# linghaosong/Sextans

Measured on AMD Instinct MI355X. Metric: SpMM GFLOP/s + achieved HBM GB/s (fp32, N=16) at 1/2/4/8 MI355X, higher is better.
Workload: dtype f32; 1 GPU; config4: synthetic CSR 4000000x4000000, Poisson(40) nnz/row, U(-1,1) fp32, N=16, alpha=0.85, beta=-2.06, column-major B/C, seed 4; M=4000000, K=4000000, N=16, nnz=159999547, parallelism=1 GPU

## Files before the change

sextans_amd/csrc/engine.hip:

```cpp
#include <algorithm>
#include <cstdlib>
#include <cstring>

#include "engine_launch.h"
#include "window_plan.h"

namespace sxe {
thread_local std::string g_last_error;
}
using namespace sxe;

namespace sxe {

int check_device(int device) {
    int n = 0;
    if (hipGetDeviceCount(&n) != hipSuccess || n <= 0) {
        g_last_error = "hipGetDeviceCount: no HIP device";
        return SEXTANS_ERR_NO_DEVICE;
    }
    if (device < 0 || device >= n) return SEXTANS_ERR_INVALID;
    hipDeviceProp_t p;
    if (hipGetDeviceProperties(&p, device) != hipSuccess) return SEXTANS_ERR_NO_DEVICE;
    if (strncmp(p.gcnArchName, "gfx950", 6) != 0) {
        g_last_error = std::string("device is ") + p.gcnArchName + ", engine is built for gfx950 only";
        return SEXTANS_ERR_NO_DEVICE;
    }
    return SEXTANS_OK;
}

enum Drops { kNothing, kWindowStream, kClusterPlan, kPackedPlans, kColwiseVerdict };
constexpr int64_t kMin = INT64_MIN, kMax = INT64_MAX;
using E = sextans_engine;
static const struct Option {
    const char *key; int64_t E::*slot; Drops drops = kNothing; bool measurement = false; int64_t lo = kMin, hi = kMax; uint64_t only = 0;
} kOptions[] = {
    {"kernel", &E::opt_kernel}, {"stage_a", &E::opt_stage}, {"xcd_remap", &E::opt_xcd}, {"exact", &E::opt_exact}, {"profile", &E::opt_profile},
    {"split_rows", &E::opt_split_rows}, {"bucket_rows", &E::opt_bucket_rows}, {"global_nnz", &E::opt_global_nnz}, {"exact_chain", &E::opt_exact_chain},
    {"fuse_b", &E::opt_fuse_b}, {"small_v2", &E::opt_small_v2}, {"colwise_tiles_adjacent", &E::opt_colwise_tiles_adjacent}, {"window_auto", &E::opt_win_auto},
    {"bell_wide", &E::opt_bell_wide}, {"bell_generation", &E::opt_bell_gen}, {"bell_shared", &E::opt_bell_shared}, {"mfma_dense_tiles", &E::opt_mfma_dense},
    {"dense_tile_fill_x100", &E::opt_dense_fill_x100},
    {"lanes_per_row", &E::opt_lpr, kNothing, false, kMin, kMax, 1 | 1 << 2 | 1 << 4 | 1 << 8},
    {"cols_per_lane", &E::opt_cols_per_lane, kNothing, false, kMin, kMax, 1 | 1 << 4 | 1 << 8},
    {"window_unroll", &E::opt_win_unroll, kNothing, false, kMin, kMax, 1 << 4 | 1 << 8},
    {"tiles_per_wg", &E::opt_tiles_per_wg, kNothing, false, 0, 1024}, {"panel_v2", &E::opt_panel_v2, kNothing, false, -1, 1},
    {"phase_timing", &E::opt_phase_timing, kNothing, true}, {"reordered_xcd", &E::opt_reordered_xcd, kNothing, true}, {"bell_debug", &E::opt_bell_debug, kNothing, true},
    {"dist_broadcast_runs", &E::opt_dist_broadcast_runs, kNothing, true}, {"rowblock_tiles", &E::opt_rb_tiles, kNothing, true},
    {"cluster_shape", &E::opt_cluster_shape, kClusterPlan, true},
    {"cluster_group", &E::opt_cluster_group, kClusterPlan, true, 1, 64},
    {"panel_min_reuse_x100", &E::opt_min_reuse_x100, kClusterPlan}, {"panel_min_reuse_wide_x100", &E::opt_min_reuse_wide_x100, kClusterPlan},
    {"row_cluster", &E::opt_row_cluster, kClusterPlan, false, -1, 2}, {"row_similarity", &E::opt_row_similarity, kClusterPlan, false, -1, 1},
    {"cluster_top", &E::opt_cluster_top, kClusterPlan}, {"small_panel", &E::opt_small_panel, kClusterPlan}, {"row_sets", &E::opt_row_sets, kClusterPlan},
    {"row_offset", &E::opt_row_offset, kClusterPlan}, {"relabel_columns", &E::opt_relabel_columns, kClusterPlan}, {"run_cluster", &E::opt_run_cluster, kClusterPlan},
    {"refine_sweeps", &E::opt_refine_sweeps, kClusterPlan}, {"refine_rows", &E::opt_refine_rows, kClusterPlan},
    {"window_rows", &E::opt_win_rows, kWindowStream, false, 1, sx::kWinMaxRowsPerWave}, {"window_cols", &E::opt_win_cols, kWindowStream, false, 1, 0x7fffffff},
    {"share_index", &E::opt_share_index, kPackedPlans}, {"split_mixed", &E::opt_split_mixed, kPackedPlans},
    {"colwise_max_len", &E::opt_colwise_max_len, kColwiseVerdict},
};

static const Option *find_option(const char *key) {
    for (const Option &o : kOptions)
        if (!strcmp(key, o.key)) return &o;
    return nullptr;
}

int transposed_options(sextans_engine *h, const char *key, int64_t value) {
    auto skip = [](const char *k) { return !strcmp(k, "row_offset") || !strcmp(k, "global_nnz"); };
    if (key) return skip(key) ? SEXTANS_OK : sextans_set_option(h->tr, key, value);
    for (const auto &o : kOptions)
        if (!skip(o.key) && h->tr->*o.slot != h->*o.slot)
            if (int rc = sextans_set_option(h->tr, o.key, h->*o.slot)) return rc;
    h->tr->opt_mode = h->opt_mode;
    return SEXTANS_OK;
}

}

extern "C" {

const char *sextans_last_error(void) { return g_last_error.c_str(); }

int sextans_device_count(int *count) {
    if (!count) return SEXTANS_ERR_INVALID;
    *count = 0;
    int n = 0;
    if (hipGetDeviceCount(&n) != hipSuccess || n <= 0) return SEXTANS_ERR_NO_DEVICE;
    int ok = 0;
    for (int d = 0; d < n; ++d)
        if (check_device(d) == SEXTANS_OK) ++ok;
    *count = ok;
    return ok > 0 ? SEXTANS_OK : SEXTANS_ERR_NO_DEVICE;
}

int sextans_create(sextans_handle_t *out, int device) {
    if (!out) return SEXTANS_ERR_INVALID;
    *out = nullptr;
    if (int rc = check_device(device)) return rc;
    SX_HIP(hipSetDevice(device));
    auto *h = new sextans_engine();
    h->device = device;
    {
        hipDeviceProp_t p;
        if (hipGetDeviceProperties(&p, device) == hipSuccess && p.multiProcessorCount > 0)
            h->num_cus = p.multiProcessorCount;
    }
    preload_device_code();
    *out = h;
    return SEXTANS_OK;
}

int sextans_destroy(sextans_handle_t h) {
    if (!h) return SEXTANS_ERR_INVALID;
    (void)hipSetDevice(h->device);
    free_matrix(h);
    free_bell(h);
    (void)hipFree(h->d_bell_Bf);
    (void)hipFree(h->d_Bp); (void)hipFree(h->d_B); (void)hipFree(h->d_Cin); (void)hipFree(h->d_Cout); (void)hipFree(h->d_Cs);
    sextans_profile_reset(h);
    (void)hipFree(h->d_P);
    if (h->ev_fork) (void)hipEventDestroy(h->ev_fork);
    if (h->ev_join) (void)hipEventDestroy(h->ev_join);
    if (h->aux_stream) (void)hipStreamDestroy(h->aux_stream);
    (void)hipFree(h->d_dbg);
    (void)hipFree(h->d_chB); (void)hipFree(h->d_chC);
    (void)hipFree(h->d_stage);
    (void)hipFree(h->d_Cfull); (void)hipFree(h->d_dist_rows); (void)hipFree(h->d_rmB); (void)hipFree(h->d_rmC);
    for (hipEvent_t e : h->dist_events) (void)hipEventDestroy(e);
    if (h->comm_stream) (void)hipStreamDestroy(h->comm_stream);
// ... 129 lines not shown
    for (int i = threadIdx.x; i < np; i += 64) {
        const int c = dict[(int64_t)(b - 1) * stride + i];
        unsigned s = ((unsigned)c * 2654435761u) >> 22;
        while (atomicCAS(&tab[s], -1, c) != -1 && tab[s] != c) s = (s + 1) & 1023u;
    }
    __syncthreads();
    unsigned found = 0;
    for (int i = threadIdx.x; i < nc; i += 64) {
        const int c = dict[(int64_t)b * stride + i];
        unsigned s = ((unsigned)c * 2654435761u) >> 22;
        while (tab[s] != -1 && tab[s] != c) s = (s + 1) & 1023u;
        found += tab[s] == c;
    }
    for (int o = 32; o > 0; o >>= 1) found += __shfl_down(found, o);
    if (threadIdx.x == 0) { atomicAdd(&out[0], (unsigned long long)found); atomicAdd(&out[1], (unsigned long long)nc); }
}
int run16_stat(sextans_engine *h, double *value) {
    *value = 0.0;
    if (h->cluster_state <= 0 || !h->d_slot_row || h->psc.plan_nblk <= 0) return SEXTANS_OK;
    const int RB = kBlock / 4 * std::max(1, h->psc.plan_sets);
    std::vector<int> sr((size_t)h->psc.plan_nblk * RB);
    SX_HIP(hipMemcpy(sr.data(), h->d_slot_row, sizeof(int) * sr.size(), hipMemcpyDeviceToHost));
    const std::vector<int> &br = h->psc.h_blk_row;
    if ((int)br.size() != h->psc.plan_nblk + 1) return SEXTANS_OK;
    int64_t in_runs = 0, slots = 0;
    for (int b = 0; b < h->psc.plan_nblk; ++b) {
        const int n = br[(size_t)b + 1] - br[(size_t)b];
        const int *r = sr.data() + (size_t)b * RB;
        slots += n;
        for (int i = 0; i < n;) {
            int j = i + 1;
            while (j < n && r[j] == r[j - 1] + 1) ++j;
            if (j - i >= 16) in_runs += j - i;
            i = j;
        }
    }
    *value = slots ? (double)in_runs / (double)slots : 0.0;
    return SEXTANS_OK;
}
int dict_overlap_stat(sextans_engine *h, double *value) {
    const sextans_engine::PanelState &P = h->cluster_state > 0 ? h->psc : h->ps;
    *value = 0.0;
    if (!P.plan_built || P.plan_nblk < 2 || !P.d_dict || !P.d_dict_ptr) return SEXTANS_OK;
    unsigned long long *d = nullptr, hv[2] = {0, 0};
    SX_HIP(hipMalloc((void **)&d, sizeof hv));
    SX_HIP(hipMemset(d, 0, sizeof hv));
    hipLaunchKernelGGL(dict_overlap, dim3((unsigned)P.plan_nblk - 1), dim3(64), 0, hipStreamPerThread, P.d_dict_ptr, P.d_dict, P.plan_dict_stride, P.plan_nblk, d);
    const hipError_t e = hipMemcpy(hv, d, sizeof hv, hipMemcpyDeviceToHost);
    (void)hipFree(d);
    SX_HIP(e);
    *value = hv[1] ? (double)hv[0] / (double)hv[1] : 0.0;
    return SEXTANS_OK;
}
}
extern "C" {

int sextans_get_stat(sextans_handle_t h, const char *key, double *value) {
    if (!h || !key || !value) return SEXTANS_ERR_INVALID;
    if (h->d_rp) {
        SX_HIP(hipSetDevice(h->device));
        if (int rc = ensure_dense(h)) return rc;
        if (int rc = ensure_split(h)) return rc;
    }
    if (!strcmp(key, "plan_build_s")) *value = h->plan_build_s;
    else if (!strcmp(key, "window_padded_entries")) *value = (double)h->win_padded;
    else if (!strcmp(key, "window_state")) *value = (double)h->win_state;
    else if (!strcmp(key, "reassociated_rows")) *value = (double)h->h_split_rows.size();
    else if (!strcmp(key, "piece_path_rows")) *value = (double)(h->nhub + h->nchain);
    else if (!strcmp(key, "exact_chain_rows")) *value = (double)h->nchain;
    else if (!strcmp(key, "chain_threshold")) *value = (double)h->chain_T;
    else if (!strcmp(key, "split_threshold")) *value = (double)h->split_T;
    else if (!strcmp(key, "bucket_threshold")) *value = (double)h->bucket_L0;
    else if (!strcmp(key, "dense_tiles")) *value = (double)h->dense_tiles;
    else if (!strcmp(key, "dense_tile_fraction")) *value = h->nnz > 0 ? (double)h->dense_nnz / (double)h->nnz : 0.0;
    else if (!strcmp(key, "dense_tiles_on_mfma")) *value = h->dense_W > 0 ? 1.0 : 0.0;
    else if (!strcmp(key, "bell_share")) *value = h->bell_share;
    else if (!strcmp(key, "row_cluster")) *value = (double)h->cluster_state;
    else if (!strcmp(key, "cluster_shared_fraction")) *value = h->cluster_shared;
    else if (!strcmp(key, "cluster_decline")) *value = (double)h->cluster_decline;
    else if (!strcmp(key, "graph_fallbacks")) *value = (double)h->graph_fallbacks;
    else if (!strcmp(key, "cluster_run16_fraction")) return run16_stat(h, value);
    else if (!strcmp(key, "dict_overlap_consecutive")) return dict_overlap_stat(h, value);
    else if (!strcmp(key, "dist_setup_exchanges")) *value = (double)h->dist_exchanges;
    else if (!strcmp(key, "cluster_graph_kind")) *value = (double)h->cluster_graph_kind;
    else if (!strcmp(key, "cluster_runs")) *value = h->cluster_runs ? 1.0 : 0.0;
    else if (!strcmp(key, "pattern_symmetry")) *value = h->pattern_symmetry;
    else if (!strcmp(key, "col_range_lo")) *value = (double)h->col_lo;
    else if (!strcmp(key, "col_range_hi")) *value = (double)h->col_hi;
    else if (!strcmp(key, "b_rows_repacked")) *value = h->d_touched ? (double)h->touched_segments * 64.0 : (double)(h->col_hi - h->col_lo);
    else if (!strcmp(key, "colwise")) *value = (double)h->colwise_state;
    else if (!strcmp(key, "mixed_plan")) *value = h->ps.plan_built && h->ps.plan_mixed ? (h->ps.d_rg_skip && h->opt_split_mixed != 0 ? 2.0 : 1.0) : 0.0;
    else if (!strcmp(key, "row_sets")) *value = (double)(h->cluster_state > 0 ? h->psc.plan_sets : h->ps.plan_sets);
    else if (!strcmp(key, "row_coherence")) *value = h->row_coherence;
    else if (!strcmp(key, "panel_blocks_clustered")) *value = (double)h->psc.plan_nblk;
    else if (!strcmp(key, "device_bytes")) *value = (double)device_bytes(h);
    else if (!strcmp(key, "softmax_long_rows")) *value = (double)h->sm_long_rows;
    else if (!strcmp(key, "value_refreshes")) *value = (double)h->value_refreshes;
    else if (!strcmp(key, "value_refresh_rebuilt")) *value = (double)h->value_refresh_rebuilt;
    else if (!strcmp(key, "bf16_native_calls")) *value = (double)(h->bf16_native_calls + (h->tr ? h->tr->bf16_native_calls : 0));
    else if (!strcmp(key, "bf16_converted_calls")) *value = (double)(h->bf16_converted_calls + (h->tr ? h->tr->bf16_converted_calls : 0));
    else if (!strcmp(key, "transpose_build_s")) *value = h->transpose_build_s + (h->tr ? h->tr->plan_build_s : 0.0);
    else if (!strcmp(key, "grid_stride_line")) *value = (double)h->cluster_s2;
    else if (!strcmp(key, "grid_stride_plane")) *value = (double)h->cluster_s3;
    else if (!strcmp(key, "panel_rows_natural")) *value = (double)h->plan_total_dict;
    else if (!strcmp(key, "panel_rows_clustered")) *value = (double)h->cluster_total_dict;
    else if (!strcmp(key, "panel_fraction")) *value = h->ps.plan_panel_frac;
    else if (!strcmp(key, "panel_blocks")) *value = (double)h->ps.plan_nblk;
    else if (!strcmp(key, "index_stream_entries")) *value = (double)(h->cluster_state > 0 ? h->psc.plan_idx_len : h->ps.plan_idx_len);
    else if (!strcmp(key, "value_stream_entries")) *value = (double)(h->cluster_state > 0 ? h->psc.plan_stream_len : h->ps.plan_stream_len);
    else return SEXTANS_ERR_INVALID;
    return SEXTANS_OK;
}

int sextans_export_plan(sextans_handle_t h, int lanes_per_row, sextans_packed *out) {
    if (!h || !out || (lanes_per_row != 2 && lanes_per_row != 4 && lanes_per_row != 8)) return SEXTANS_ERR_INVALID;
    if (!h->d_rp) return SEXTANS_ERR_STATE;
    SX_HIP(hipSetDevice(h->device));
    if (int rc = ensure_dense(h)) return rc;
    if (int rc = ensure_split(h)) return rc;
    if (int rc = ensure_plan(h, lanes_per_row, true)) return rc;
    if (!h->ps.plan_built) return SEXTANS_ERR_STATE;
    if (int rc = restore_plan_streams(h)) return rc;
    const auto &ps = h->ps;
    const int M = h->M, nblk = ps.plan_nblk, RB = kBlock / lanes_per_row;
    const size_t L = (size_t)ps.plan_stream_len;
    memset(out, 0, sizeof *out);
    out->M = M; out->K = h->K; out->nnz = h->m_nnz; out->lanes_per_row = lanes_per_row; out->nblk = nblk;
    out->stream_len = (int64_t)L; out->max_dict = ps.plan_max_dict; out->nnz_in_panel_blocks = ps.plan_nnz_panel;
    std::vector<int> rp((size_t)M + 1), cnt((size_t)nblk), bd((size_t)nblk * ps.plan_dict_stride);
    SX_HIP(hipMemcpy(rp.data(), h->m_rp, sizeof(int) * rp.size(), hipMemcpyDeviceToHost));
    if (nblk) {
        SX_HIP(hipMemcpy(cnt.data(), ps.d_dict_ptr, sizeof(int) * cnt.size(), hipMemcpyDeviceToHost));
        SX_HIP(hipMemcpy(bd.data(), ps.d_dict, sizeof(int) * bd.size(), hipMemcpyDeviceToHost));
    }
#define SX_HIP_OUT(call) do { if ((call) != hipSuccess) { g_last_error = #call; (void)hipGetLastError(); sextans_packed_free(out); return SEXTANS_ERR_HIP; } } while (0)
    auto alloc = [](size_t bytes) { return calloc(bytes ? bytes : 1, 1); };
    out->blk_row = (int *)alloc(sizeof(int) * ((size_t)nblk + 1));
    out->dict_ptr = (int *)alloc(sizeof(int) * ((size_t)nblk + 1));
    out->row_off = (int *)alloc(sizeof(int) * ((size_t)M + 1));
    out->idx16 = (uint16_t *)alloc(sizeof(uint16_t) * L);
    out->col32 = (int *)alloc(sizeof(int) * L);
    out->val = (float *)alloc(sizeof(float) * L);
    size_t ndict = 0;
    for (int b = 0; b < nblk; ++b) ndict += (size_t)cnt[(size_t)b];
    out->dict = (int *)alloc(sizeof(int) * ndict);
    if (!out->blk_row || !out->dict_ptr || !out->row_off || !out->idx16 || !out->col32 || !out->val || !out->dict) {
        sextans_packed_free(out);
        return SEXTANS_ERR_ALLOC;
    }
    memcpy(out->blk_row, ps.h_blk_row.data(), sizeof(int) * ((size_t)nblk + 1));
    size_t w = 0;
    for (int b = 0; b < nblk; ++b) {
        out->dict_ptr[b] = (int)w;
        for (int i = 0; i < cnt[(size_t)b]; ++i) out->dict[w++] = bd[(size_t)b * ps.plan_dict_stride + (size_t)i];
    }
    out->dict_ptr[nblk] = (int)w;
    for (int r = 0; r < M; ++r) out->row_off[r + 1] = out->row_off[r] + ((rp[(size_t)r + 1] - rp[(size_t)r] + 3) & ~3);
    if (!ps.d_ioff) {
        SX_HIP_OUT(hipMemcpy(out->idx16, ps.d_lidx, sizeof(uint16_t) * L, hipMemcpyDeviceToHost));
    } else {
        std::vector<uint16_t> comp((size_t)ps.plan_idx_len);
        std::vector<int> ioff((size_t)nblk * RB * 2), sinfo((size_t)nblk * RB * 2);
        SX_HIP_OUT(hipMemcpy(comp.data(), ps.d_lidx, sizeof(uint16_t) * comp.size(), hipMemcpyDeviceToHost));
        SX_HIP_OUT(hipMemcpy(ioff.data(), ps.d_ioff, sizeof(int) * ioff.size(), hipMemcpyDeviceToHost));
        SX_HIP_OUT(hipMemcpy(sinfo.data(), ps.d_row_off, sizeof(int) * sinfo.size(), hipMemcpyDeviceToHost));
        const unsigned pad = (unsigned)ps.plan_pad_row * 16u * (unsigned)lanes_per_row;
// ... 113 lines not shown
```

sextans_amd/csrc/engine_dist.hip:

```cpp
#include <dlfcn.h>

#include <algorithm>
#include <cstring>
#include <mutex>

#include "engine_launch.h"

using namespace sxe;

namespace sxe {
namespace {
__global__ __launch_bounds__(256) void position_rows(int nblk, int RB, const int *__restrict__ blk_row, const int *__restrict__ slot_row, int row0, int *__restrict__ out) {
    const int b = blockIdx.x, s = threadIdx.x;
    if (b >= nblk || s >= RB) return;
    const int p0 = blk_row[b], n = blk_row[b + 1] - p0;
    if (s < n) out[p0 + s] = slot_row[(int64_t)b * RB + s] + row0;
}
}

static bool cc_usable(sextans_engine *h, int N, const Tiling &t) {
    return h->cluster_state == 2 && h->cluster_cm_pays && t.W == 16 && N % 16 == 0 && t.segs.size() == 1 && t.segs[0].width == 16 && h->nhub == 0 &&
           h->nchain == 0 && csr_only(h) && (h->opt_kernel == 0 || h->opt_kernel == 2) && h->d_Cs && h->d_slot_row &&
           h->Cs_cap >= (size_t)(N / 16) * (size_t)h->M * 16 && h->Bp_cap >= (size_t)h->K * (size_t)N && h->psc.plan_sets == 1 &&
           (h->M >= 65536 || h->m_nnz * (int64_t)N >= ((int64_t)24 << 20)) && (int)h->psc.h_blk_row.size() == h->psc.plan_nblk + 1;
// ... 98 lines not shown
    if (i < m.y) C[(int64_t)m.x + i + (int64_t)n * ldc] = S[((int64_t)g * N + n) * lmax + i];
}

int exchange(sextans_engine *h, Rccl *r, void *comm, int world, int rank, const int *mine, int n, std::vector<int> &all, int status, hipStream_t s,
             const char *what) {
    ++h->dist_exchanges;
    const size_t per = (size_t)n + 1;
    std::vector<int> me(per, 0), buf(per * (size_t)world, 0);
    for (int i = 0; i < n; ++i) me[(size_t)i] = status ? 0 : mine[i];
    me[(size_t)n] = status;
    int *d = nullptr;
    SX_HIP(hipMalloc((void **)&d, sizeof(int) * buf.size()));
    hipError_t e0 = hipMemcpyAsync(d + per * (size_t)rank, me.data(), sizeof(int) * per, hipMemcpyHostToDevice, s);
    const int rc = e0 != hipSuccess ? SEXTANS_OK : rccl_check(r->AllGather(d + per * (size_t)rank, d, per, 2 , comm, s), what);
    hipError_t e1 = (rc || e0 != hipSuccess) ? hipSuccess : hipMemcpyAsync(buf.data(), d, sizeof(int) * buf.size(), hipMemcpyDeviceToHost, s);
    hipError_t e2 = hipStreamSynchronize(s);
    (void)hipFree(d);
    if (rc) return rc;
    SX_HIP(e0);
    SX_HIP(e1);
    SX_HIP(e2);
    bool peer_failed = false;
    all.assign((size_t)n * (size_t)world, 0);
    for (int g = 0; g < world; ++g) {
        peer_failed = peer_failed || buf[per * (size_t)g + (size_t)n] != 0;
        for (int i = 0; i < n; ++i) all[(size_t)g * n + (size_t)i] = buf[per * (size_t)g + (size_t)i];
    }
    if (status) return status;
    if (peer_failed) {
        g_last_error = std::string(what) + ": another rank reported a failure";
        return SEXTANS_ERR_PEER;
    }
    return SEXTANS_OK;
}

struct Partition {
    int64_t M_total = 0;
    int row0 = 0, m_loc = 0, m_max = 0;
    bool equal = true;
};
int read_partition(int world, int rank, const int *row_ranges, int multiple_of, Partition &p) {
    p = Partition();
    for (int g = 0; g < world; ++g) {
        if (row_ranges[2 * g] != (int)p.M_total || row_ranges[2 * g + 1] < row_ranges[2 * g] || (row_ranges[2 * g + 1] % multiple_of)) return SEXTANS_ERR_INVALID;
        p.M_total = row_ranges[2 * g + 1];
        p.m_max = std::max(p.m_max, row_ranges[2 * g + 1] - row_ranges[2 * g]);
        p.equal = p.equal && row_ranges[2 * g + 1] - row_ranges[2 * g] == row_ranges[1] - row_ranges[0];
    }
    p.row0 = row_ranges[2 * rank];
    p.m_loc = row_ranges[2 * rank + 1] - p.row0;
    return SEXTANS_OK;
}

int exchange_nnz(sextans_engine *h, Rccl *r, void *comm, int world, int rank, const int *row_ranges, bool force, int status, hipStream_t s, bool *exchanged) {
    if (!comm) return status;
    std::vector<int> nnz_key(row_ranges, row_ranges + 2 * world);
    nnz_key.push_back(rank);
    if (!force && h->dist_nnz_key == nnz_key) return status;
    const int mine_nz[2] = {(int)(h->nnz & 0x7fffffff), (int)(h->nnz >> 31)};
    std::vector<int> all_nz;
    *exchanged = true;
    if (int rc = exchange(h, r, comm, world, rank, mine_nz, 2, all_nz, status, s, "ncclAllGather(nnz)")) return rc;
    int64_t total = 0;
    for (int g = 0; g < world; ++g) total += (int64_t)all_nz[2 * (size_t)g] + ((int64_t)all_nz[2 * (size_t)g + 1] << 31);
    if (total != h->opt_global_nnz)
        if (int rc = sextans_set_option(h, "global_nnz", total)) return rc;
    h->dist_nnz_key = nnz_key;
    return SEXTANS_OK;
}

int settle(sextans_engine *h, Rccl *r, void *comm, int world, int rank, int status, bool exchanged, hipStream_t s) {
    if (!comm || !exchanged) return status;
    std::vector<int> none;
    const int rc = exchange(h, r, comm, world, rank, nullptr, 0, none, status, s, "ncclAllGather(status)");
    if (rc) { h->dist_cut_key.clear(); h->dist_nnz_key.clear(); }
    return rc;
}

struct CmSetup {
    Partition p;
    std::vector<int64_t> lmax, off;
    int *d_meta = nullptr;
    bool cc = false;
};
int setup_cm(sextans_engine *h, Rccl *r, void *comm, int world, int rank, const int *row_ranges, int N, int &nchunks, hipStream_t s, bool force, CmSetup &out) {
    bool exchanged = false;
    int st = read_partition(world, rank, row_ranges, 1, out.p);
    const Partition &p = out.p;
    if (!st && p.m_loc != h->M) st = SEXTANS_ERR_INVALID;
    if (!st && !h->d_rp) st = SEXTANS_ERR_STATE;
    if (st && !(force && comm)) return st;
    if (!st && world > 1 && h->opt_row_offset != p.row0) st = sextans_set_option(h, "row_offset", p.row0);
    if (nchunks < 1) nchunks = 1;
    if (nchunks > 16) nchunks = 16;
    if (int rc = exchange_nnz(h, r, comm, world, rank, row_ranges, force, st, s, &exchanged)) return rc;
    bool want_cc = false;
    if (nchunks > 1) {
        st = cc_prepare(h, N, &want_cc);
    } else if (h->M > 0) {
        st = prepare(h, N);
    }
    if (want_cc && h->psc.plan_nblk < nchunks) want_cc = false;
    std::vector<int> key(row_ranges, row_ranges + 2 * world);
    key.push_back(N); key.push_back(nchunks); key.push_back(rank); key.push_back(want_cc ? 1 : 0);
    if (force || h->dist_cut_key != key || st) {
        h->dist_cut_key.clear();
        const size_t need = (size_t)world * (size_t)p.m_max;
        if (!st && want_cc && h->dist_rows_cap < need) {
            (void)hipFree(h->d_dist_rows);
            h->d_dist_rows = nullptr; h->dist_rows_cap = 0;
            if (hipMalloc((void **)&h->d_dist_rows, sizeof(int) * std::max<size_t>(need, 1)) != hipSuccess) { (void)hipGetLastError(); st = SEXTANS_ERR_HIP; g_last_error = "hipMalloc(row tables) failed"; }
            else h->dist_rows_cap = need;
        }
        bool all_cc = want_cc && !st;
        if (comm) {
            const int mine_f = want_cc ? 1 : 0;
            std::vector<int> f;
            exchanged = true;
            if (int rc = exchange(h, r, comm, world, rank, &mine_f, 1, f, st, s, "ncclAllGather(mode)")) return rc;
            for (int g = 0; g < world; ++g) all_cc = all_cc && f[(size_t)g] != 0;
        } else if (st) {
            return st;
        }
        h->dist_cc = all_cc;
        if (all_cc) {
            cc_table(h, p.row0, h->d_dist_rows + (size_t)rank * p.m_max, s);
            if (comm)
                if (int rc = rccl_check(r->AllGather(h->d_dist_rows + (size_t)rank * p.m_max, h->d_dist_rows, (size_t)p.m_max, 2 , comm, s),
                                        "ncclAllGather(row tables)"))
                    return rc;
            ++h->dist_exchanges;
            SX_HIP(hipStreamSynchronize(s));
        }
        std::vector<int> mine((size_t)nchunks + 1, 0);
        mine[(size_t)nchunks] = p.m_loc;
        for (int c = 1; c < nchunks && !st; ++c) {
            if (all_cc) {
                mine[(size_t)c] = h->psc.h_blk_row[(size_t)((int64_t)h->psc.plan_nblk * c / nchunks)];
                continue;
            }
            int a = (int)((int64_t)p.m_loc * c / nchunks);
            st = sextans_align_row(h, N, a, &a);
            mine[(size_t)c] = std::min(std::max(a, mine[(size_t)c - 1]), p.m_loc);
        }
        std::vector<int> all;
        if (!comm) {
            if (st) return st;
            all = mine;
        } else {
            exchanged = true;
            if (int rc = exchange(h, r, comm, world, rank, mine.data(), nchunks + 1, all, st, s, "ncclAllGather(cuts)")) return rc;
        }
        for (int g = 0; g < world && !st; ++g) {
            const int len = row_ranges[2 * g + 1] - row_ranges[2 * g];
            const int *cg = all.data() + (size_t)g * (nchunks + 1);
            if (cg[0] != 0 || cg[nchunks] != len) st = SEXTANS_ERR_STATE;
            for (int c = 0; c < nchunks && !st; ++c)
                if (cg[c + 1] < cg[c]) st = SEXTANS_ERR_STATE;
        }
        if (!st) { h->dist_cuts = all; h->dist_cut_key = key; }
    }
    auto workspaces = [&]() -> int {
        auto cut = [&](int g, int c) { return h->dist_cuts[(size_t)g * (nchunks + 1) + (size_t)c]; };
        out.lmax.assign((size_t)nchunks, 1);
        out.off.assign((size_t)nchunks + 1, 0);
        for (int c = 0; c < nchunks; ++c) {
            for (int g = 0; g < world; ++g) out.lmax[(size_t)c] = std::max<int64_t>(out.lmax[(size_t)c], cut(g, c + 1) - cut(g, c));
            out.off[(size_t)c + 1] = out.off[(size_t)c] + (int64_t)world * N * out.lmax[(size_t)c];
        }
        const size_t meta_floats = (size_t)nchunks * (size_t)world * 2;
        if (h->stage_cap < (size_t)out.off[(size_t)nchunks] + meta_floats) h->dist_meta_at = nullptr;
        if (int rc = ensure(&h->d_stage, &h->stage_cap, (size_t)out.off[(size_t)nchunks] + meta_floats)) return rc;
        if (!h->comm_stream) SX_HIP(hipStreamCreateWithFlags(&h->comm_stream, hipStreamNonBlocking));
        while (h->dist_events.size() < (size_t)nchunks + 1) {
            hipEvent_t e;
            SX_HIP(hipEventCreateWithFlags(&e, hipEventDisableTiming));
            h->dist_events.push_back(e);
        }
        std::vector<int> meta(meta_floats);
        for (int c = 0; c < nchunks; ++c)
            for (int g = 0; g < world; ++g) {
                meta[((size_t)c * world + g) * 2] = row_ranges[2 * g] + cut(g, c);
                meta[((size_t)c * world + g) * 2 + 1] = cut(g, c + 1) - cut(g, c);
            }
        out.d_meta = reinterpret_cast<int *>(h->d_stage + out.off[(size_t)nchunks]);
        if (h->dist_meta != meta || h->dist_meta_at != out.d_meta) {
            SX_HIP(hipMemcpyAsync(out.d_meta, meta.data(), sizeof(int) * meta.size(), hipMemcpyHostToDevice, s));
            ++h->dist_exchanges;
            SX_HIP(hipStreamSynchronize(s));
            h->dist_meta = meta;
            h->dist_meta_at = out.d_meta;
        }
        out.cc = h->dist_cc;
        if (out.cc)
            if (int rc = ensure(&h->d_Cfull, &h->Cfull_cap, (size_t)p.M_total * (size_t)N)) return rc;
        return SEXTANS_OK;
    };
    if (!st) st = workspaces();
    return settle(h, r, comm, world, rank, st, exchanged, s);
}

int setup_rm(sextans_engine *h, Rccl *r, void *comm, int world, int rank, const int *row_ranges, int N, bool packed, hipStream_t s, bool force, Partition &p) {
    bool exchanged = false;
    int st = read_partition(world, rank, row_ranges, 1, p);
    if (!st && p.m_loc != h->M) st = SEXTANS_ERR_INVALID;
    if (!st && !h->d_rp) st = SEXTANS_ERR_STATE;
    if (st && !(force && comm)) return st;
    if (!st && world > 1 && h->opt_row_offset != p.row0) st = sextans_set_option(h, "row_offset", p.row0);
    if (int rc = exchange_nnz(h, r, comm, world, rank, row_ranges, force, st, s, &exchanged)) return rc;
    if (force && h->M > 0)
        st = rm_plan(h, N, s);
    if (!st && packed && comm) {
        st = ensure(&h->d_stage, &h->stage_cap, (size_t)p.M_total * (size_t)N);
        h->dist_meta_at = nullptr;
    }
    return settle(h, r, comm, world, rank, st, exchanged || (force && comm), s);
}

struct BellSetup {
    Partition p;
    int64_t lmax = 1;
    size_t slab = 0;
    int *d_meta = nullptr;
};
int setup_bell(sextans_engine *h, Rccl *r, void *comm, int world, int rank, const int *row_ranges, int N, hipStream_t s, bool force, BellSetup &out) {
    int st = read_partition(world, rank, row_ranges, 32, out.p);
    const Partition &p = out.p;
    if (!st && p.m_loc != h->bell_M) st = SEXTANS_ERR_INVALID;
    if (!st && !h->d_bell_Af) st = SEXTANS_ERR_STATE;
    if (st && !(force && comm)) return st;
    auto workspaces = [&]() -> int {
        out.lmax = std::max<int64_t>(1, p.m_max);
        out.slab = (size_t)N * (size_t)out.lmax;
        const size_t meta_floats = (size_t)world * 2;
        if (h->stage_cap < (size_t)world * out.slab + meta_floats) h->dist_meta_at = nullptr;
        if (int rc = ensure(&h->d_stage, &h->stage_cap, (size_t)world * out.slab + meta_floats)) return rc;
        std::vector<int> meta(meta_floats);
        for (int g = 0; g < world; ++g) { meta[2 * (size_t)g] = row_ranges[2 * g]; meta[2 * (size_t)g + 1] = row_ranges[2 * g + 1] - row_ranges[2 * g]; }
        out.d_meta = reinterpret_cast<int *>(h->d_stage + (size_t)world * out.slab);
        if (h->dist_meta != meta || h->dist_meta_at != out.d_meta) {
            SX_HIP(hipMemcpyAsync(out.d_meta, meta.data(), sizeof(int) * meta.size(), hipMemcpyHostToDevice, s));
            ++h->dist_exchanges;
            SX_HIP(hipStreamSynchronize(s));
            h->dist_meta = meta;
            h->dist_meta_at = out.d_meta;
        }
        return SEXTANS_OK;
    };
    if (!st) st = workspaces();
    return settle(h, r, comm, world, rank, st, force && comm, s);
}

int dist_args_ok(sextans_handle_t h, void *comm, int world, int rank, const int *row_ranges) {
    return h && (comm || world == 1) && world >= 1 && rank >= 0 && rank < world && row_ranges;
}
}

extern "C" {

int sextans_dist_bind_library(const char *path) {
    std::lock_guard<std::mutex> lk(g_bind_mutex);
    if (g_live_comms > 0) {
        g_last_error = "sextans_dist_bind_library: communicators of the current library are still alive";
        return SEXTANS_ERR_STATE;
    }
    g_bind_path = path && *path ? path : "";
    rccl_bind_locked();
    g_bound = true;
    if (!g_r.lib) { g_last_error = g_rccl_error; return SEXTANS_ERR_STATE; }
    return SEXTANS_OK;
}

int sextans_dist_unique_id(char id[128]) {
    if (!id) return SEXTANS_ERR_INVALID;
    Rccl *r = rccl();
    if (!r) return SEXTANS_ERR_STATE;
    return rccl_check(r->GetUniqueId(id), "ncclGetUniqueId");
}

int sextans_dist_comm_init(void **comm, int device, int world, int rank, const char id[128]) {
    if (!comm || !id || world < 1 || rank < 0 || rank >= world) return SEXTANS_ERR_INVALID;
    if (int rc = check_device(device)) return rc;
    Rccl *r = rccl();
    if (!r) return SEXTANS_ERR_STATE;
    SX_HIP(hipSetDevice(device));
    Id128 u;
    memcpy(u.b, id, 128);
    { std::lock_guard<std::mutex> lk(g_bind_mutex); ++g_live_comms; }
    const int rc = rccl_check(r->CommInitRank(comm, world, u, rank), "ncclCommInitRank");
    if (rc) { std::lock_guard<std::mutex> lk(g_bind_mutex); --g_live_comms; }
    return rc;
}

int sextans_dist_comm_destroy(void *comm) {
    Rccl *r = rccl();
    if (!r || !comm) return SEXTANS_ERR_INVALID;
    const int rc = rccl_check(r->CommDestroy(comm), "ncclCommDestroy");
    std::lock_guard<std::mutex> lk(g_bind_mutex);
    if (g_live_comms > 0) --g_live_comms;
    return rc;
}

int sextans_dist_prepare(sextans_handle_t h, void *comm, int world, int rank, const int *row_ranges, int N, int nchunks, int form, void *stream) {
    if (!dist_args_ok(h, comm, world, rank, row_ranges) || N <= 0) return SEXTANS_ERR_INVALID;
    if (form != SEXTANS_DIST_CSR_COLMAJOR && form != SEXTANS_DIST_CSR_ROWMAJOR && form != SEXTANS_DIST_BELL) return SEXTANS_ERR_INVALID;
    if (N % (form == SEXTANS_DIST_BELL ? 32 : 8)) return SEXTANS_ERR_INVALID;
    Rccl *r = comm ? rccl() : nullptr;
    if (comm && !r) return SEXTANS_ERR_STATE;
    SX_HIP(hipSetDevice(h->device));
    hipStream_t s = (hipStream_t)stream;
    if (form == SEXTANS_DIST_CSR_COLMAJOR) {
        CmSetup cs;
        return setup_cm(h, r, comm, world, rank, row_ranges, N, nchunks, s, true, cs);
    }
    if (form == SEXTANS_DIST_CSR_ROWMAJOR) {
        Partition p;
        return setup_rm(h, r, comm, world, rank, row_ranges, N, nchunks < 0, s, true, p);
    }
    BellSetup bs;
    return setup_bell(h, r, comm, world, rank, row_ranges, N, s, true, bs);
}

int sextans_dist_spmm(sextans_handle_t h, void *comm, int world, int rank, const int *row_ranges, int N, float alpha,
                      const float *d_B, int64_t ldb, float beta, const float *d_C_in, int64_t ldc_in, float *d_C_out,
                      int64_t ldc, int nchunks, void *stream) {
    if (!dist_args_ok(h, comm, world, rank, row_ranges) || N <= 0 || (N % 8) || !d_B || !d_C_in || !d_C_out) return SEXTANS_ERR_INVALID;
    if (!h->d_rp) return SEXTANS_ERR_STATE;
    Rccl *r = comm ? rccl() : nullptr;
    if (comm && !r) return SEXTANS_ERR_STATE;
    SX_HIP(hipSetDevice(h->device));
    hipStream_t s = (hipStream_t)stream;
    CmSetup cs;
    if (int rc = setup_cm(h, r, comm, world, rank, row_ranges, N, nchunks, s, false, cs)) return rc;
    const Partition &p = cs.p;
    const int64_t M_total = p.M_total;
    const int row0 = p.row0, m_max = p.m_max;
    if (ldc < M_total || ldc_in < M_total || ldb < h->K) return SEXTANS_ERR_INVALID;
    auto cut = [&](int g, int c) { return h->dist_cuts[(size_t)g * (nchunks + 1) + (size_t)c]; };
    const std::vector<int64_t> &lmax = cs.lmax, &off = cs.off;
    int *d_meta = cs.d_meta;
    const bool cc = cs.cc;
    bool first = true;
    for (int c = 0; c < nchunks; ++c) {
        float *S = h->d_stage + off[(size_t)c];
        const int c0 = cut(rank, c), c1 = cut(rank, c + 1);
        float *mine = S + (size_t)rank * N * lmax[(size_t)c];
        if (cc) {
            if (first) cc_pre(h, N, d_B, ldb, d_C_in + row0, ldc_in, s);
            first = false;
            const int b0 = (int)((int64_t)h->psc.plan_nblk * c / nchunks), b1 = c + 1 == nchunks ? h->psc.plan_nblk : (int)((int64_t)h->psc.plan_nblk * (c + 1) / nchunks);
            if (int rc = cc_chunk(h, N, alpha, beta, b0, b1, h->d_dist_rows + (size_t)rank * m_max, row0, mine, lmax[(size_t)c], s)) return rc;
        } else if (c1 > c0) {
            if (int rc = sextans_spmm_device_rows(h, N, alpha, d_B, ldb, beta, d_C_in + row0 + c0, ldc_in, mine,
                                                  lmax[(size_t)c], c0, c1, first ? 0 : SEXTANS_ROWS_REUSE_B_PANELS, stream))
                return rc;
            first = false;
        }
        SX_HIP(hipEventRecord(h->dist_events[(size_t)c], s));
        SX_HIP(hipStreamWaitEvent(h->comm_stream, h->dist_events[(size_t)c], 0));
        if (comm)
            if (int rc = rccl_check(r->AllGather(mine, S, (size_t)N * (size_t)lmax[(size_t)c], 7 , comm,
                                                 h->comm_stream), "ncclAllGather"))
                return rc;
        if (cc) {
            for (int g = 0; g < world; ++g)
                launch_slab_rows(true, h->d_Cfull, M_total * 16, h->d_dist_rows + (size_t)g * m_max + cut(g, c), 0, cut(g, c + 1) - cut(g, c),
                                 S + (size_t)g * N * lmax[(size_t)c], lmax[(size_t)c] * 16, N / 16, h->comm_stream);
            continue;
        }
        const unsigned gx = (unsigned)((lmax[(size_t)c] + 255) / 256);
        hipLaunchKernelGGL(dist_unpack_slabs, dim3(gx, (unsigned)N, (unsigned)world), dim3(256), 0, h->comm_stream, S,
                           lmax[(size_t)c], N, reinterpret_cast<const int2 *>(d_meta) + (size_t)c * world, d_C_out, ldc);
    }
    if (cc) launch_tiles_to_colmajor(h->d_Cfull, d_C_out, ldc, (int)M_total, 0, N / 16, N, h->comm_stream);
    SX_HIP(hipEventRecord(h->dist_events[(size_t)nchunks], h->comm_stream));
    SX_HIP(hipStreamWaitEvent(s, h->dist_events[(size_t)nchunks], 0));
    SX_HIP(hipGetLastError());
    return SEXTANS_OK;
}

int sextans_dist_spmm_rm(sextans_handle_t h, void *comm, int world, int rank, const int *row_ranges, int N, float alpha, const float *d_B,
                         int64_t ldb, float beta, const float *d_C_in, int64_t ldc_in, float *d_C_out, int64_t ldc, void *stream) {
    if (!dist_args_ok(h, comm, world, rank, row_ranges) || N <= 0 || (N % 8) || !d_B || !d_C_in || !d_C_out || ldb < N || ldc_in < N || ldc < N)
        return SEXTANS_ERR_INVALID;
    if (!h->d_rp) return SEXTANS_ERR_STATE;
    Rccl *r = comm ? rccl() : nullptr;
    if (comm && !r) return SEXTANS_ERR_STATE;
    SX_HIP(hipSetDevice(h->device));
    hipStream_t s = (hipStream_t)stream;
    const bool packed = ldc != N;
    Partition p;
    if (int rc = setup_rm(h, r, comm, world, rank, row_ranges, N, packed, s, false, p)) return rc;
    const int64_t M_total = p.M_total;
    const int row0 = p.row0, m_loc = p.m_loc;
    const bool equal = p.equal && h->opt_dist_broadcast_runs == 0;
    if (comm && !equal && (!r->Broadcast || !r->GroupStart || !r->GroupEnd)) {
        g_last_error = "RCCL library lacks ncclBroadcast / ncclGroupStart / ncclGroupEnd (row ranges of unequal length)";
        return SEXTANS_ERR_STATE;
    }
    if (m_loc > 0)
        if (int rc = sextans_spmm_device_rm(h, N, alpha, d_B, ldb, beta, d_C_in + (int64_t)row0 * ldc_in, ldc_in, d_C_out + (int64_t)row0 * ldc, ldc, stream))
            return rc;
    if (!comm) return SEXTANS_OK;
    float *X = d_C_out;
    if (packed) {
        X = h->d_stage;
        if (m_loc > 0)
            SX_HIP(hipMemcpy2DAsync(X + (int64_t)row0 * N, sizeof(float) * (size_t)N, d_C_out + (int64_t)row0 * ldc, sizeof(float) * (size_t)ldc, sizeof(float) * (size_t)N,
                                    (size_t)m_loc, hipMemcpyDeviceToDevice, s));
    }
    if (equal) {
        const size_t count = (size_t)m_loc * (size_t)N;
        if (int rc = rccl_check(r->AllGather(X + (size_t)rank * count, X, count, 7 , comm, s), "ncclAllGather(row-major C)")) return rc;
    } else {
        if (int rc = rccl_check(r->GroupStart(), "ncclGroupStart")) return rc;
        int rc = SEXTANS_OK;
        for (int g = 0; g < world && rc == SEXTANS_OK; ++g) {
            const size_t count = (size_t)(row_ranges[2 * g + 1] - row_ranges[2 * g]) * (size_t)N;
            float *run = X + (int64_t)row_ranges[2 * g] * N;
            if (count) rc = rccl_check(r->Broadcast(run, run, count, 7 , g, comm, s), "ncclBroadcast(row-major C)");
        }
        const int rc2 = rccl_check(r->GroupEnd(), "ncclGroupEnd");
        if (rc) return rc;
        if (rc2) return rc2;
    }
// ... 35 lines not shown
```

sextans_amd/csrc/engine_state.h:

```cpp
#pragma once
#include <hip/hip_runtime.h>

#include <chrono>
#include <cstdint>
#include <cstdio>
#include <set>
#include <string>
#include <vector>

#include "sextans_amd.h"
#include "thread_stream.h"

namespace sxe {
extern thread_local std::string g_last_error;
}

#define SX_HIP(call)                                                                    \
    do {                                                                                \
        hipError_t e_ = (call);                                                         \
        if (e_ != hipSuccess) {                                                         \
            char buf_[512];                                                             \
            snprintf(buf_, sizeof buf_, "%s failed: %s (%s:%d)", #call,                 \
                     hipGetErrorString(e_), __FILE__, __LINE__);                        \
            sxe::g_last_error = buf_;                                                   \
// ... 95 lines not shown
    int64_t cluster_s2 = 0, cluster_s3 = 0;
    int64_t plan_total_dict = 0, cluster_total_dict = 0;
    PanelState plan_stash[3];
    uint2 *d_wstream = nullptr;
    int *d_wstep0 = nullptr;
    int win_nwaves = 0, win_rw = 0;
    int64_t win_padded = 0;
    int win_state = 0;
    int64_t win_built_rows = -1, win_built_cols = -1;
    double plan_build_s = 0.0;
    int dense_mb = 0, dense_W = 0;
    double dense_share = 0.0;
    int dense_max_union = 0;
    int *d_dense_col = nullptr;
    void *d_dense_Af = nullptr;
    int64_t dense_tiles = 0, dense_nnz = 0;
    int64_t dense_built_mfma = -2, dense_built_fill = -2;
    int rb_n = 0;
    int64_t rb_groups = 0;
    int *d_rb_row0 = nullptr, *d_rb_gptr = nullptr, *d_rb_gcol = nullptr;
    float *d_rb_A = nullptr;
    int sb_n = 0;
    int64_t sb_entries = 0;
    int *d_sb_uptr = nullptr, *d_sb_ucol = nullptr;
    unsigned char *d_sb_umask = nullptr;
    int bell_M = 0, bell_K = 0, bell_W = 0;
    int bell_max_union = 0;
    double bell_share = 0.0;
    const int *d_bell_col = nullptr;
    int *d_bell_col_owned = nullptr;
    void *d_bell_Af = nullptr;
    void *d_bell_Bf = nullptr;
    size_t bell_Bf_cap = 0;
    const int *s_rp = nullptr, *s_ci = nullptr;
    const float *s_v = nullptr;
    int64_t s_nnz = 0;
    int *d_srp = nullptr, *d_sci = nullptr;
    float *d_sv = nullptr;
    const int *m_rp = nullptr, *m_ci = nullptr;
    const float *m_v = nullptr;
    int64_t m_nnz = 0;
    int *d_mrp = nullptr, *d_mci = nullptr;
    float *d_mv = nullptr;
    unsigned char *d_skip = nullptr;
    struct PieceTable {
        int *d_vrp = nullptr, *d_vend = nullptr, *d_vfirst = nullptr, *d_row = nullptr;
        std::vector<int> h_row, h_vfirst;
    };
    PieceTable by_len, by_row;
    int nchain = 0;
    int *d_chain_row = nullptr, *d_chain_beg = nullptr, *d_chain_perm = nullptr;
    long long *d_chain_off = nullptr;
    int *d_chain_ci_perm = nullptr, *d_chain_beg_c = nullptr;
    float *d_chain_v_c = nullptr;
    std::vector<int> h_chain_row;
    std::vector<long long> h_chain_off;
    int64_t chain_T = 0;
    int64_t chain_built_opt = -2;
    hipStream_t aux_stream = nullptr;
    hipEvent_t ev_fork = nullptr, ev_join = nullptr;
    std::vector<int> h_split_rows;
    int nhub = 0;
    int split_nv = 0;
    int64_t split_T = 0, bucket_L0 = 0;
    int64_t split_built_opt = -2, bucket_built_opt = -2, split_built_gnnz = -2;
    float *d_P = nullptr;
    size_t P_cap = 0;
    long long *d_dbg = nullptr;
    float *d_stage = nullptr;
    size_t stage_cap = 0;
    int64_t graph_fallbacks = 0;
    hipStream_t comm_stream = nullptr;
    std::vector<hipEvent_t> dist_events;
    float *d_rmB = nullptr, *d_rmC = nullptr;
    size_t rmB_cap = 0, rmC_cap = 0;
    float *d_bfB = nullptr, *d_bfC = nullptr;
    size_t bfB_cap = 0, bfC_cap = 0;
    int64_t bf16_native_calls = 0, bf16_converted_calls = 0;
    float *d_Cfull = nullptr;
    size_t Cfull_cap = 0;
    int *d_dist_rows = nullptr;
    size_t dist_rows_cap = 0;
    bool dist_cc = false;
    int64_t dist_exchanges = 0;
    std::vector<int> dist_nnz_key;
    std::vector<int> dist_cut_key, dist_cuts;
    std::vector<int> dist_meta;
    const int *dist_meta_at = nullptr;
    int64_t opt_share_index = 1;
    int64_t opt_refine_rows = 62;
    int64_t opt_refine_sweeps = 8;
    int64_t opt_run_cluster = 0;
    int64_t opt_reordered_xcd = -1;
    int64_t opt_row_similarity = -1;
    int64_t opt_relabel_columns = 1;
    int64_t opt_colwise_tiles_adjacent = 1;
    int64_t opt_split_mixed = 1;
    int64_t opt_small_panel = 1;
    int64_t opt_cluster_top = 1 << 30;
    int64_t opt_colwise_max_len = 6;
    int64_t opt_kernel = 0, opt_lpr = 0, opt_stage = 1, opt_xcd = 1, opt_exact = 1, opt_profile = 0;
    int64_t opt_cols_per_lane = 0;
    int64_t opt_cluster_shape = 0;
    int64_t opt_cluster_group = 6;
    int64_t opt_row_cluster = -1;
    int64_t opt_row_offset = -1;
    int64_t opt_row_sets = 2;
    int64_t opt_small_v2 = 1;
    int64_t opt_panel_v2 = -1;
    int64_t opt_tiles_per_wg = 0;
    int64_t opt_fuse_b = 1;
    int64_t opt_split_rows = 0;
    int64_t opt_global_nnz = 0;
    int64_t opt_exact_chain = 1;
    int64_t opt_bucket_rows = -1;
    int64_t opt_phase_timing = 0;
    int64_t opt_min_reuse_x100 = 200;
    int64_t opt_min_reuse_wide_x100 = 150;
    int64_t opt_win_rows = 319;
    int64_t opt_win_cols = 65536;
    int64_t opt_win_unroll = 8;
    int64_t opt_win_auto = 0;
    int64_t opt_bell_shared = -1;
    int64_t opt_rb_tiles = 0;
    int64_t opt_mode = 0;
    int64_t opt_dist_broadcast_runs = 0;
    int64_t opt_bell_debug = 0;
    int64_t opt_bell_gen = 0;
    int64_t opt_bell_wide = 1;
    int64_t opt_mfma_dense = 0;
    int64_t opt_dense_fill_x100 = 50;
    std::vector<sxe::EventPair> ev_kernel, ev_repack, ev_post;
    const char *last_kernel = "none";
    std::string last_kernel_buf;
    sextans_engine *tr = nullptr;
    int *d_trp = nullptr, *d_tci = nullptr;
    float *d_tv = nullptr;
    int *d_tperm = nullptr;
    double transpose_build_s = 0.0;
    int *d_sddmm_row0 = nullptr;
    int64_t sddmm_row0_n = 0;
    int *d_sm_wrow = nullptr;
    int64_t sm_wrow_n = 0;
    int2 *d_sm_tab = nullptr;
    float2 *d_sm_part = nullptr;
    int sm_nchunks = 0, sm_long_rows = 0;
};

namespace sxe {

int check_device(int device);
void free_panel_state(sextans_engine::PanelState &p);
void free_plan(sextans_engine *h);
void free_cluster_plan(sextans_engine *h);
int64_t plan_key(const sextans_engine *h);
int64_t device_bytes(const sextans_engine *h);
void free_window(sextans_engine *h);
void free_bell(sextans_engine *h);
void free_split(sextans_engine *h);
void free_dense(sextans_engine *h);
void free_matrix(sextans_engine *h);
void free_backward(sextans_engine *h);
int validate_matrix(sextans_engine *h);
void free_softmax(sextans_engine *h);
int ensure_softmax_tables(sextans_engine *h, hipStream_t s);
int prepare_transposed(sextans_engine *h, int N, hipStream_t s);
int transposed_options(sextans_engine *h, const char *key, int64_t value);
int ensure(float **p, size_t *cap, size_t need);
int allow_big_lds(sextans_engine *h, const void *kern, int bytes);
int read_back_row_ptr(sextans_engine *h, std::vector<int> &rp, int level = 2);
int read_back_entries(sextans_engine *h, std::vector<int> &ci, std::vector<float> &va, int level = 2);
int ensure_plan(sextans_engine *h, int lpr, bool force);
int ensure_cluster_plan(sextans_engine *h);
int restore_plan_streams(sextans_engine *h);
int ensure_colwise(sextans_engine *h);
int ensure_col_range(sextans_engine *h);
int ensure_window(sextans_engine *h, bool force);
bool window_pays(const sextans_engine *h, int N, int64_t padded);
int ensure_split(sextans_engine *h);
int ensure_dense(sextans_engine *h);
int prepare(sextans_engine *h, int N, bool whole = true, Tiling *out = nullptr);
inline bool colwise_wanted(const sextans_engine *h) { return h->opt_kernel == 4 || (h->opt_kernel == 0 && h->colwise_state == 1); }
inline bool csr_only(const sextans_engine *h) { return h->dense_W == 0 && h->rb_n == 0; }
int launch_dense_tiles(sextans_engine *h, int N, float alpha, const float *d_B, int64_t ldb, float beta, const float *d_C_in,
                       int64_t ldc_in, float *d_C_out, int64_t ldc, hipStream_t s);
int launch_rowblocks(sextans_engine *h, const std::vector<Seg> &plan, const float *d_C_in, int64_t ldc_in, float *d_C_out, int64_t ldc, int N, int row_begin,
                     int row_end, float alpha, float beta, hipStream_t s);
int mark_rowblock_skip(sextans_engine *h);

int rm_plan(sextans_engine *h, int N, hipStream_t s, Tiling *out = nullptr);
int check_rm_bf16_args(sextans_handle_t h, int N, const uint16_t *d_B, int64_t ldb, const void *d_C_in, int64_t ldc_in, void *d_C_out, int64_t ldc, int c_dtype);
int fork_chains(sextans_engine *h, const Call &c, const std::vector<Seg> &segs, int ch0, int ch1, bool rm);
void cc_table(sextans_engine *h, int row0, int *d_out, hipStream_t s);

template <class T>
int upload(T **dst, const std::vector<T> &src) {
    SX_HIP(hipMalloc((void **)dst, sizeof(T) * (src.empty() ? 1 : src.size())));
    if (!src.empty()) SX_HIP(hipMemcpy(*dst, src.data(), sizeof(T) * src.size(), hipMemcpyHostToDevice));
    return SEXTANS_OK;
}

struct PlanTimer {
    sextans_engine *h; std::chrono::steady_clock::time_point t0 = std::chrono::steady_clock::now();
    explicit PlanTimer(sextans_engine *h_) : h(h_) {}
    ~PlanTimer() { h->plan_build_s += std::chrono::duration<double>(std::chrono::steady_clock::now() - t0).count(); }
};

struct Prof {
    sextans_engine *h; std::vector<EventPair> *vec; hipStream_t s; bool on; EventPair ep{};
// ... 13 lines not shown
```

Measured before the change: 1636 GFLOP/s.

## Exchange distributed C column runs directly via per-column broadcasts, skipping staging

Adds a default-on direct path for distributed SpMM. Each rank computes its row chunks straight into the output C, and an RCCL group of per-column broadcasts (or all-gathers) on a comm stream then exchanges the rows in place, replacing the packed staging buffer and the unpack step. This is meant to cut staging copies and workspace setup while still overlapping communication with compute per chunk. The cost is many small collectives (one per column per rank), which may add latency. The measured config runs on one GPU, so it only skips workspace setup there.

```diff
diff --git a/sextans_amd/csrc/engine.hip b/sextans_amd/csrc/engine.hip
--- a/sextans_amd/csrc/engine.hip
+++ b/sextans_amd/csrc/engine.hip
@@ -43,6 +43,7 @@
     {"cols_per_lane", &E::opt_cols_per_lane, kNothing, false, kMin, kMax, 1 | 1 << 4 | 1 << 8},
     {"window_unroll", &E::opt_win_unroll, kNothing, false, kMin, kMax, 1 << 4 | 1 << 8},
     {"tiles_per_wg", &E::opt_tiles_per_wg, kNothing, false, 0, 1024}, {"panel_v2", &E::opt_panel_v2, kNothing, false, -1, 1},
+    {"dist_direct", &E::opt_dist_direct, kNothing, false, 0, 1},
     {"phase_timing", &E::opt_phase_timing, kNothing, true}, {"reordered_xcd", &E::opt_reordered_xcd, kNothing, true}, {"bell_debug", &E::opt_bell_debug, kNothing, true},
     {"dist_broadcast_runs", &E::opt_dist_broadcast_runs, kNothing, true}, {"rowblock_tiles", &E::opt_rb_tiles, kNothing, true},
     {"cluster_shape", &E::opt_cluster_shape, kClusterPlan, true},
@@ -338,6 +339,7 @@
     else if (!strcmp(key, "cluster_run16_fraction")) return run16_stat(h, value);
     else if (!strcmp(key, "dict_overlap_consecutive")) return dict_overlap_stat(h, value);
     else if (!strcmp(key, "dist_setup_exchanges")) *value = (double)h->dist_exchanges;
+    else if (!strcmp(key, "dist_direct")) *value = (double)h->dist_direct_last;
     else if (!strcmp(key, "cluster_graph_kind")) *value = (double)h->cluster_graph_kind;
     else if (!strcmp(key, "cluster_runs")) *value = h->cluster_runs ? 1.0 : 0.0;
     else if (!strcmp(key, "pattern_symmetry")) *value = h->pattern_symmetry;
diff --git a/sextans_amd/csrc/engine_dist.hip b/sextans_amd/csrc/engine_dist.hip
--- a/sextans_amd/csrc/engine_dist.hip
+++ b/sextans_amd/csrc/engine_dist.hip
@@ -204,6 +204,7 @@
     std::vector<int64_t> lmax, off;
     int *d_meta = nullptr;
     bool cc = false;
+    bool direct = false;
 };
 int setup_cm(sextans_engine *h, Rccl *r, void *comm, int world, int rank, const int *row_ranges, int N, int &nchunks, hipStream_t s, bool force, CmSetup &out) {
     bool exchanged = false;
@@ -284,6 +285,18 @@
     }
     auto workspaces = [&]() -> int {
         auto cut = [&](int g, int c) { return h->dist_cuts[(size_t)g * (nchunks + 1) + (size_t)c]; };
+        out.cc = h->dist_cc;
+        out.direct = h->opt_dist_direct != 0 && !out.cc && (!comm || (r->Broadcast && r->GroupStart && r->GroupEnd));
+        if (out.direct) {
+            if (!comm) return SEXTANS_OK;
+            if (!h->comm_stream) SX_HIP(hipStreamCreateWithFlags(&h->comm_stream, hipStreamNonBlocking));
+            while (h->dist_events.size() < (size_t)nchunks + 1) {
+                hipEvent_t e;
+                SX_HIP(hipEventCreateWithFlags(&e, hipEventDisableTiming));
+                h->dist_events.push_back(e);
+            }
+            return SEXTANS_OK;
+        }
         out.lmax.assign((size_t)nchunks, 1);
         out.off.assign((size_t)nchunks + 1, 0);
         for (int c = 0; c < nchunks; ++c) {
@@ -313,7 +326,6 @@
             h->dist_meta = meta;
             h->dist_meta_at = out.d_meta;
         }
-        out.cc = h->dist_cc;
         if (out.cc)
             if (int rc = ensure(&h->d_Cfull, &h->Cfull_cap, (size_t)p.M_total * (size_t)N)) return rc;
         return SEXTANS_OK;
@@ -463,6 +475,49 @@
     int *d_meta = cs.d_meta;
     const bool cc = cs.cc;
     bool first = true;
+    h->dist_direct_last = cs.direct ? 1 : 0;
+    if (cs.direct) {
+        const bool gather = nchunks == 1 && p.equal && h->opt_dist_broadcast_runs == 0;
+        const bool exchange = comm && world > 1;
+        for (int c = 0; c < nchunks; ++c) {
+            const int c0 = cut(rank, c), c1 = cut(rank, c + 1);
+            if (c1 > c0) {
+                if (int rc = sextans_spmm_device_rows(h, N, alpha, d_B, ldb, beta, d_C_in + row0 + c0, ldc_in, d_C_out + row0 + c0, ldc, c0, c1,
+                                                      first ? 0 : SEXTANS_ROWS_REUSE_B_PANELS, stream))
+                    return rc;
+                first = false;
+            }
+            if (!exchange) continue;
+            SX_HIP(hipEventRecord(h->dist_events[(size_t)c], s));
+            SX_HIP(hipStreamWaitEvent(h->comm_stream, h->dist_events[(size_t)c], 0));
+            bool any = false;
+            for (int g = 0; g < world; ++g) any = any || cut(g, c + 1) > cut(g, c);
+            if (!any) continue;
+            if (int rc = rccl_check(r->GroupStart(), "ncclGroupStart")) return rc;
+            int rc = SEXTANS_OK;
+            for (int n = 0; n < N && rc == SEXTANS_OK; ++n) {
+                float *col = d_C_out + (int64_t)n * ldc;
+                if (gather) {
+                    rc = rccl_check(r->AllGather(col + (int64_t)rank * p.m_loc, col, (size_t)p.m_loc, 7 , comm, h->comm_stream), "ncclAllGather(column of C)");
+                    continue;
+                }
+                for (int g = 0; g < world && rc == SEXTANS_OK; ++g) {
+                    const size_t count = (size_t)(cut(g, c + 1) - cut(g, c));
+                    float *run = col + row_ranges[2 * g] + cut(g, c);
+                    if (count) rc = rccl_check(r->Broadcast(run, run, count, 7 , g, comm, h->comm_stream), "ncclBroadcast(column run of C)");
+                }
+            }
+            const int rc2 = rccl_check(r->GroupEnd(), "ncclGroupEnd");
+            if (rc) return rc;
+            if (rc2) return rc2;
+        }
+        if (exchange) {
+            SX_HIP(hipEventRecord(h->dist_events[(size_t)nchunks], h->comm_stream));
+            SX_HIP(hipStreamWaitEvent(s, h->dist_events[(size_t)nchunks], 0));
+        }
+        SX_HIP(hipGetLastError());
+        return SEXTANS_OK;
+    }
     for (int c = 0; c < nchunks; ++c) {
         float *S = h->d_stage + off[(size_t)c];
         const int c0 = cut(rank, c), c1 = cut(rank, c + 1);
diff --git a/sextans_amd/csrc/engine_state.h b/sextans_amd/csrc/engine_state.h
--- a/sextans_amd/csrc/engine_state.h
+++ b/sextans_amd/csrc/engine_state.h
@@ -201,6 +201,7 @@
     int *d_dist_rows = nullptr;
     size_t dist_rows_cap = 0;
     bool dist_cc = false;
+    int dist_direct_last = 0;
     int64_t dist_exchanges = 0;
     std::vector<int> dist_nnz_key;
     std::vector<int> dist_cut_key, dist_cuts;
@@ -244,6 +245,7 @@
     int64_t opt_rb_tiles = 0;
     int64_t opt_mode = 0;
     int64_t opt_dist_broadcast_runs = 0;
+    int64_t opt_dist_direct = 1;
     int64_t opt_bell_debug = 0;
     int64_t opt_bell_gen = 0;
     int64_t opt_bell_wide = 1;
```

After: 1634 GFLOP/s. Within noise of the previous version (-0.1%).
